# deep-privacy/sidekit

Hardware: AMD Instinct MI355X
Metric: x-vectors/sec (4 s @ 16 kHz) (higher is better)
Workload: dtype bf16; 1 GPU; HalfResNet34 Xtractor.submit / collect (2 whole batches in flight; each batch is the forward of Xtractor.forward(is_eval=True)), bf16 trunk, batch=256 per GPU, synthetic 4 s @ 16 kHz (BASELINE.json configs[1]); batch_per_gpu=256, samples_per_utt=64000, frames_per_utt=401, resident_input_batches=5, parallelism=utterance-sharded x1, lanes=1

## Files before the change

### sidekit_amd/csrc/conv3x3.hip

```cpp
#include "kernels.h"

namespace sk {

template <typename T> __device__ inline void mma_step(f32x16& acc, const uint4& w, const uint4& x);

template <> __device__ inline void mma_step<bf16_t>(f32x16& acc, const uint4& w, const uint4& x) {
  acc = __builtin_amdgcn_mfma_f32_32x32x16_bf16(__builtin_bit_cast(bf16x8, w), __builtin_bit_cast(bf16x8, x), acc, 0, 0, 0);
}
template <> __device__ inline void mma_step<float>(f32x16& acc, const uint4& w, const uint4& x) {
  acc = __builtin_amdgcn_mfma_f32_32x32x2f32(__builtin_bit_cast(float, w.x), __builtin_bit_cast(float, x.x), acc, 0, 0, 0);
  acc = __builtin_amdgcn_mfma_f32_32x32x2f32(__builtin_bit_cast(float, w.y), __builtin_bit_cast(float, x.y), acc, 0, 0, 0);
  acc = __builtin_amdgcn_mfma_f32_32x32x2f32(__builtin_bit_cast(float, w.z), __builtin_bit_cast(float, x.z), acc, 0, 0, 0);
  acc = __builtin_amdgcn_mfma_f32_32x32x2f32(__builtin_bit_cast(float, w.w), __builtin_bit_cast(float, x.w), acc, 0, 0, 0);
}

enum { LANES_LINEAR = 0, LANES_GRID = 1, LANES_DENSE = 2 };
template <typename T_, int CIN_, int COUT_, int S_, int WIN_, int TH_, int WM_, int WN_, int MW_, int NW_, int CK_, int TAPS_, int OCC_ = 0, int PD_ = 0, bool SWZ_ = false, int BLK_ = LANES_LINEAR, bool M16_ = false, bool DIRECT_ = false, bool S2G_ = false, int LEANF_ = -1>
struct ConvCfg {
  static constexpr bool DIRECT = DIRECT_;
  static_assert(!DIRECT_ || (!M16_), "DIRECT: 32x32 MFMA accumulator layout");
  using T = T_;
  static constexpr int EB = elem<T_>::bytes;
  static constexpr int CIN = CIN_, COUT = COUT_, S = S_, WIN = WIN_, TH = TH_, WM = WM_, WN = WN_, MW = MW_, NW = NW_, CK = CK_;
  static constexpr int TAPS = TAPS_;
  static constexpr int WOUT = WIN / S;
  static constexpr int MT = TH * WOUT;
  static constexpr int NT = WN * NW * 32;
  static constexpr int RIN = (TH - 1) * S + 3;
  static constexpr int WP = WIN + 2;
  static constexpr int CB = CK * EB;
  static constexpr bool SWZ = SWZ_;
  static constexpr int BLK = BLK_;
  static constexpr int GC = BLK == LANES_GRID ? (WIN_ / S_) / MW_ : 16, GR = 16 / GC;
  static_assert(BLK == LANES_LINEAR || (SWZ_ && S_ == 1 && TAPS_ == 9), "block lane orders: swizzled image, stride 1, 3x3");
  static_assert(BLK != LANES_GRID || (GC * MW_ == WIN_ / S_ && GR * GC == 16 && TH_ == 2 * WM_ * GR), "GRID: W = MW * GC, TH = 2 * WM * GR");
  static_assert(BLK != LANES_DENSE || (WM_ == 1 && CK_ * elem<T_>::bytes == 256 && TH_ * (WIN_ + 1) <= MW_ * 32), "DENSE: 256-B positions, one wave row");
  static constexpr bool M16 = M16_;
  static_assert(!M16 || ((BLK != LANES_LINEAR || S2G_) && elem<T_>::bytes == 2 && (CK_ * 2) % 64 == 0), "M16: bf16, block lane orders (or the planar stride-2 image), 64-B k-steps");
  static constexpr bool LEAD = BLK == LANES_DENSE || (BLK == LANES_GRID && CK_ * elem<T_>::bytes < 256);
  static constexpr int IMG0 = LEAD ? CK_ * elem<T_>::bytes : 0;
  static constexpr int PSTRIDE = SWZ ? CB : CB + 16;
  static constexpr int SPP = PSTRIDE / 16;
  static constexpr int PPR = ((SWZ ? WIN : WP) * SPP + 63) / 64;
  static constexpr int RS = SWZ ? (WIN + 1) * CB : PPR * 1024;
  static constexpr int LDS_SWZ = (RIN - 1) * RS + (PPR * 1024 > RS ? PPR * 1024 : RS);
  static constexpr int LDS_BLK = BLK == LANES_DENSE ? IMG0 + (MW * 32 + 2 * (WIN + 1) + 2) * CB : IMG0 + LDS_SWZ;
  static constexpr int LDS_IN = BLK ? (LDS_BLK + 255) / 256 * 256 : (SWZ ? (LDS_SWZ + 255) / 256 * 256 : RIN * RS);
  static constexpr int LDS_OUT = TH_ * (WIN_ / S_) * (WN_ * 32 * elem<T_>::bytes + 16);
  static constexpr int LDS = LDS_IN > LDS_OUT ? LDS_IN : (LDS_OUT + 255) / 256 * 256;
  static constexpr int SWF = SPP < 16 ? SPP : 16;
  static constexpr int SWSH = SPP == 4 ? 2 : (SPP == 8 ? 1 : 0);
  static constexpr int KCMASK = (GC >> SWSH) - 1;
  static constexpr int KRSH = SWSH == 0 ? (GC == 4 ? 2 : (GC == 8 ? 3 : 4)) : (SWSH == 1 ? (GC == 8 ? 2 : 3) : 2);
  static constexpr bool S2G = S2G_;
  static constexpr int S2GR = S2G_ ? TH_ / WM_ : 1, S2GC = 16 / S2GR, S2NBC = (WIN_ / S_) / S2GC;
  static constexpr int S2PPB = 256 / (CK_ * elem<T_>::bytes) > 0 ? 256 / (CK_ * elem<T_>::bytes) : 1;
  static constexpr int S2PB = S2GC / S2PPB > 0 ? S2GC / S2PPB : 1;
  static_assert(!S2G_ || (BLK_ == LANES_LINEAR && SWZ_ && S_ == 2 && TAPS_ == 9 && TH_ % WM_ == 0 && S2GR * S2GC == 16 &&
                          (WIN_ / 2) % S2GC == 0 && 2 * MW_ >= S2NBC && S2GC >= S2PPB && S2GR * S2PB == CK_ * elem<T_>::bytes / 16),
                "S2G: stride 2, swizzled image, 16-position blocks that tile the output rows, one key value per slot of a position");
  __host__ __device__ static constexpr int planar(int col) { return (col < 0 || col >= WIN) ? WIN : (col & 1) * (WIN / 2) + (col >> 1); }
  __host__ __device__ static constexpr int unplanar(int P) { return P < WIN / 2 ? 2 * P : 2 * (P - WIN / 2) + 1; }
  __host__ __device__ static constexpr int s2_rowkey(int row) {
    const int hp = (row >> 1) & (S2GR - 1);
    return ((M16_ && S2GR == 8) ? (((hp << 1) & 7) | (hp >> 2)) : hp) * S2PB;
  }
  __host__ __device__ static constexpr int s2p_half(int p) { return (p >= 4 && p < 12) ? 1 : 0; }
  __host__ __device__ static constexpr int s2p_j(int p) { return p < 4 ? p : (p < 12 ? p - 4 : p - 8); }
  __host__ __device__ static constexpr int s2p_row(int p) { return S2GR == 8 ? 2 * (s2p_j(p) / S2GC) + s2p_half(p) : s2p_half(p) * (S2GR / 2) + s2p_j(p) / S2GC; }
  __host__ __device__ static constexpr int s2p_col(int p) { return s2p_j(p) % S2GC; }
  static constexpr int PT16 = S2G_ ? S2NBC : 2 * MW_;
  __host__ __device__ static constexpr int swz_key(int row, int col) {
    if (S2G) return s2_rowkey(row) | ((col / S2PPB) & (S2PB - 1));
    if (BLK == LANES_GRID) return (((row & (GR - 1)) << KRSH) | ((col >> SWSH) & KCMASK)) & (SWF - 1);
    if (BLK == LANES_DENSE) return dense_key((row * (WIN + 1) + col) & 15);
    return (col >> SWSH) & (SWF - 1);
  }
  __host__ __device__ static constexpr int dense_key(int x) { return (M16_ && BLK_ == LANES_DENSE) ? (((x & 7) << 1) | (x >> 3)) : x; }
  __host__ __device__ static constexpr int p16_row(int p) { return GR == 2 ? ((p >= 4 && p < 12) ? 1 : 0) : p / GC; }
  __host__ __device__ static constexpr int p16_col(int p) { return GR == 2 ? (p < 4 ? p : (p < 12 ? p - 4 : p - 8)) : p % GC; }
  __host__ __device__ static constexpr int p16_dense(int p) { return p < 8 ? p : (p < 12 ? p + 4 : p - 4); }
  static_assert(!SWZ || (SPP == 4 || SPP == 8 || SPP == 16 || SPP == 32), "swizzled image: 64..512 B per position");
  static constexpr int KS = CB / 32;
  static constexpr int NCH = CIN / CK;
  static constexpr int KTOT = NCH * TAPS * KS;
  static constexpr int OCC = OCC_ ? OCC_ : ((MW * NW <= 5 && 160 * 1024 / LDS * WM * WN >= 8) ? 2 : 1);
  static constexpr int NK = TAPS * KS;
  static constexpr int KS32 = CB / 64, NK32 = TAPS * KS32, KTOT32 = NCH * NK32;
  static constexpr int MT16 = 2 * MW, NT16 = 2 * NW;
  static constexpr int PD = PD_ ? PD_ : ((NK * NW <= 24) ? NK : (NW == 1 ? 8 : 4));
  static constexpr int PD16 = NK32 * NT16 <= 18 ? NK32 : (PD_ >= 16 ? PD_ - 16 : 2);
  static constexpr bool RESIDENT = TAPS == 9 && NCH == 1 && (M16 ? PD16 == NK32 : PD == NK) && NT == COUT;
  static constexpr bool LEAN = LEANF_ < 0 ? (RESIDENT || OCC >= 3) : (LEANF_ != 0);
  static_assert(MT <= WM * MW * 32, "positions must be covered by the waves' 32-row MFMA tiles (trailing tiles may be partial or idle)");
  static constexpr bool PARTIAL_M = MT < WM * MW * 32;
  __device__ static inline int lane_pos16(int wm, int t, int p) {
    if constexpr (S2G) {
      return t < S2NBC ? (wm * S2GR + s2p_row(p)) * WOUT + t * S2GC + s2p_col(p) : MT;
    } else if constexpr (BLK == LANES_GRID) {
      return ((2 * wm + t / MW) * GR + p16_row(p)) * WOUT + (t % MW) * GC + p16_col(p);
    } else {
      const int L = t * 16 + p16_dense(p), row = L / (WIN + 1), col = L % (WIN + 1);
      return (col < WIN && row < TH) ? row * WOUT + col : MT;
    }
  }
  __device__ static inline int lane_pos(int wm, int i, int r) {
    if constexpr (BLK == LANES_GRID) {
      const int g = ((r >= 4 && r < 12) || (r >= 16 && r < 20) || r >= 28) ? 1 : 0;
      const int j = r - (r < 4 ? 0 : (r < 12 ? 4 : (r < 20 ? 8 : (r < 28 ? 12 : 16))));
      return ((2 * wm + g) * GR + j / GC) * WOUT + i * GC + j % GC;
    } else if constexpr (BLK == LANES_DENSE) {
      const int L = i * 32 + r, row = L / (WIN + 1), col = L % (WIN + 1);
      return (col < WIN && row < TH) ? row * WOUT + col : MT;
    } else if constexpr (S2G) {
      const int g = ((r >= 4 && r < 12) || (r >= 16 && r < 20) || r >= 28) ? 1 : 0;
      const int j = r - (r < 4 ? 0 : (r < 12 ? 4 : (r < 20 ? 8 : (r < 28 ? 12 : 16))));
      const int bc = 2 * i + g;
      return bc < S2NBC ? (wm * S2GR + j / S2GC) * WOUT + bc * S2GC + j % S2GC : MT;
    } else {
      return (wm * MW + i) * 32 + r;
    }
  }
  static_assert(COUT % NT == 0 && CIN % CK == 0 && CB % 32 == 0, "channel tiling");
  static_assert(LDS <= 160 * 1024, "LDS budget");
};

enum { FORM_PLAIN = 0, FORM_STATS = 1, FORM_RESID = 2, FORM_RESID_SC = 3 };
template <int F> struct FormTag { static constexpr int value = F; };

template <class C, int FORM>
__global__ __launch_bounds__(C::WM * C::WN * 64, C::OCC)
void conv3x3_kernel(ConvArgs a) {
  using T = typename C::T;
  constexpr int NWAVES = C::WM * C::WN, NTHREADS = NWAVES * 64;
  constexpr int NY = C::COUT / C::NT;
  const int bidx = NY == 1 ? (int)blockIdx.x : (int)(((blockIdx.x >> 3) / NY) * 8 + (blockIdx.x & 7));
  const int nt0 = (NY == 1 ? 0 : (int)((blockIdx.x >> 3) % NY)) * (C::NT / 32);
  __shared__ __attribute__((aligned(1024))) unsigned char smem[C::LDS];
  const int tid = threadIdx.x, lane = tid & 63, wave = __builtin_amdgcn_readfirstlane(tid >> 6);
  const int r = lane & 31, h = lane >> 5;
  const int wm = __builtin_amdgcn_readfirstlane(wave / C::WN), wn = __builtin_amdgcn_readfirstlane(wave % C::WN);
  const int tiles = (a.Hout + C::TH - 1) / C::TH;
  const int nwork = a.B * tiles, q8 = nwork >> 3, r8 = nwork & 7, xcd = bidx & 7;
  const int wfirst = xcd < r8 ? xcd * (q8 + 1) : r8 * (q8 + 1) + (xcd - r8) * q8, wcount = q8 + (xcd < r8 ? 1 : 0);
  const int wstride = (int)(gridDim.x >> 3) + (xcd < (int)(gridDim.x & 7) ? 1 : 0);
  auto stamp = [&](int k) {
    if (a.stamps && tid == 0) {
      unsigned long long* sp = a.stamps + (size_t)bidx * 8;
      sp[k] = __builtin_amdgcn_s_memtime();
      if (k == 0) sp[7] = __builtin_amdgcn_s_memrealtime();
      if (k == 6) sp[7] = __builtin_amdgcn_s_memrealtime() - sp[7];
    }
  };

  int base[C::BLK ? 1 : C::MW][C::SWZ ? 3 : 1];
  constexpr int NTR = (C::BLK == LANES_GRID && C::GR >= 4) ? 3 : 1;
  int tapreg[C::BLK == LANES_GRID ? NTR : 1][3];
  int fixreg = 0;
  if constexpr (C::BLK == LANES_GRID && C::M16) {
    const int p = lane & 15, q = lane >> 4;
    const int row0 = C::p16_row(p), col0 = C::p16_col(p);
    const int lanebase = (2 * wm * C::GR + row0) * C::RS + col0 * C::CB;
#pragma unroll
    for (int t = 0; t < NTR; ++t)
#pragma unroll
      for (int dw = 0; dw < 3; ++dw) tapreg[t][dw] = lanebase + ((C::swz_key(row0 + t, col0 + dw - 1) ^ q) << 4);
    if constexpr (!C::LEAD) fixreg = col0 == 0 ? C::RS - C::CB : -C::CB;
  } else if constexpr (C::BLK == LANES_GRID) {
    const int g = ((r >= 4 && r < 12) || (r >= 16 && r < 20) || r >= 28) ? 1 : 0;
    const int j = r - (r < 4 ? 0 : (r < 12 ? 4 : (r < 20 ? 8 : (r < 28 ? 12 : 16))));
    const int row0 = (2 * wm + g) * C::GR + j / C::GC, col0 = j % C::GC;
    const int lanebase = row0 * C::RS + col0 * C::CB;
#pragma unroll
    for (int t = 0; t < NTR; ++t)
#pragma unroll
      for (int dw = 0; dw < 3; ++dw) tapreg[t][dw] = lanebase + ((C::swz_key(row0 + t, col0 + dw - 1) ^ h) << 4);
    if constexpr (!C::LEAD) fixreg = col0 == 0 ? C::RS - C::CB : -C::CB;
  }
  int s2x = 0;
  int s2b[3] = {0, 0, 0}, s2bz = 0;
  if constexpr (C::S2G && C::M16) {
    const int p = lane & 15, q = lane >> 4;
    const int ho = wm * C::S2GR + C::s2p_row(p), pcol = C::s2p_col(p);
    s2x = (C::s2_rowkey(2 * ho) ^ C::s2_rowkey(2 * ho + 2)) << 4;
#pragma unroll
    for (int dw = 0; dw < 3; ++dw) {
      const int P = dw == 1 ? pcol : C::WIN / 2 + pcol - (dw == 0 ? 1 : 0);
      s2b[dw] = (2 * ho) * C::RS + P * C::CB + ((q ^ C::swz_key(2 * ho, P)) << 4);
    }
    const int Pz = pcol == 0 ? C::WIN : C::WIN / 2 + pcol - 1;
    s2bz = (2 * ho) * C::RS + Pz * C::CB + ((q ^ C::swz_key(2 * ho, Pz)) << 4);
  }
  if constexpr (C::S2G && !C::M16) {
    const int g = ((r >= 4 && r < 12) || (r >= 16 && r < 20) || r >= 28) ? 1 : 0;
    const int j = r - (r < 4 ? 0 : (r < 12 ? 4 : (r < 20 ? 8 : (r < 28 ? 12 : 16))));
    const int ho = wm * C::S2GR + j / C::S2GC;
    s2x = (C::s2_rowkey(2 * ho) ^ C::s2_rowkey(2 * ho + 2)) << 4;
#pragma unroll
    for (int i = 0; i < C::MW; ++i) {
      const int bc = 2 * i + g < C::S2NBC ? 2 * i + g : C::S2NBC - 1;
      const int wo = bc * C::S2GC + j % C::S2GC;
#pragma unroll
      for (int dw = 0; dw < 3; ++dw) {
        const int P = C::planar(2 * wo + dw - 1);
        base[i][dw] = (2 * ho) * C::RS + P * C::CB + ((h ^ C::swz_key(2 * ho, P)) << 4);
      }
    }
  }
#pragma unroll
  for (int i = 0; i < ((C::BLK || C::S2G) ? 0 : C::MW); ++i) {
    const int mraw = (wm * C::MW + i) * 32 + r, m = (C::PARTIAL_M && mraw >= C::MT) ? C::MT - 1 : mraw;
    const int ho = m / C::WOUT, wo = m % C::WOUT;
    if constexpr (C::SWZ) {
#pragma unroll
      for (int dw = 0; dw < 3; ++dw) {
        int col = wo * C::S + dw - 1;
        if (col < 0) col = C::WIN;
        const int f = (col >> C::SWSH) & (C::SWF - 1);
        base[i][dw] = (ho * C::S) * C::RS + col * C::CB + ((h ^ f) << 4);
      }
    } else {
      base[i][0] = (ho * C::S) * C::RS + (wo * C::S) * C::PSTRIDE + h * 16;
    }
  }
  const unsigned char* wbase = reinterpret_cast<const unsigned char*>(a.wpack);
  const unsigned lane16 = (unsigned)lane * 16u;
  auto wload = [&](int j, int kidx) {
    const unsigned soff = (unsigned)__builtin_amdgcn_readfirstlane(((nt0 + j * C::WN + wn) * C::KTOT + kidx) * 1024);
    return *reinterpret_cast<const uint4*>(wbase + soff + lane16);
  };
  const unsigned char* in = reinterpret_cast<const unsigned char*>(a.in);

  constexpr int NK = C::NK, PD = C::PD;
  constexpr bool RESIDENT = C::RESIDENT;
  auto kord = [](int kk) {
    return (C::SWZ && C::TAPS == 9 && !C::BLK) ? ((kk % 3) * 3 + kk / (3 * C::KS)) * C::KS + (kk / 3) % C::KS : kk;
  };
  uint4 wq[C::M16 ? 1 : PD][C::NW];
  constexpr int PD16 = C::PD16, NK32 = C::NK32;
  uint4 wq16[C::M16 ? PD16 : 1][C::M16 ? C::NT16 : 1];
  auto wload16 = [&](int jn, int kidx32) {
    const unsigned soff = (unsigned)__builtin_amdgcn_readfirstlane(((2 * (nt0 + (jn >> 1) * C::WN + wn) + (jn & 1)) * C::KTOT32 + kidx32) * 1024);
    return *reinterpret_cast<const uint4*>(wbase + soff + lane16);
  };
  auto load_weights = [&](int ch) {
// ... 28 lines not shown
#pragma unroll
  for (int i = 0; i < C::MW; ++i)
#pragma unroll
    for (int j = 0; j < C::NW; ++j)
#pragma unroll
      for (int q = 0; q < 16; ++q) acc[i][j][q] = 0.f;

  for (int ch = 0; ch < C::NCH; ++ch) {
    if constexpr (!RESIDENT) load_weights(ch);
    __builtin_amdgcn_sched_barrier(0);
    if (ch) __syncthreads();
    constexpr int CPP = C::CB / 16, NPIECE = C::RIN * C::PPR;
    if constexpr (C::SWZ) {
      if (ch == 0) {
        for (int s = tid; s < C::RIN * C::SPP; s += NTHREADS)
          *reinterpret_cast<uint4*>(smem + C::IMG0 + (s / C::SPP) * C::RS + C::WIN * C::CB + (s % C::SPP) * 16) = make_uint4(0, 0, 0, 0);
        if constexpr (C::LEAD) {
          if (tid < C::SPP) *reinterpret_cast<uint4*>(smem + tid * 16) = make_uint4(0, 0, 0, 0);
        }
      }
    }
    for (int it = (a.dbg & 4) ? NPIECE : wave; it < NPIECE; it += NWAVES) {
      const int row = it / C::PPR, q = it % C::PPR;
      const int hi = hi0 + row;
      const bool rowok = hi >= 0 && hi < hin_b;
      const unsigned char* rowbase = in + ((((size_t)b * a.Hin + hi) * C::WIN) * C::CIN + ch * C::CK) * C::EB;
      const int slot = q * 64 + lane;
      const unsigned char* src = reinterpret_cast<const unsigned char*>(a.zeros);
      if constexpr (C::SWZ) {
        const int col = slot / C::SPP, cs = slot % C::SPP;
        const int cc = cs ^ C::swz_key(row, col);
        if (rowok) src = rowbase + (C::S2G ? C::unplanar(col) : col) * (C::CIN * C::EB) + cc * 16;
        if ((C::WIN * C::SPP) % 64 == 0 || slot < C::WIN * C::SPP)
          __builtin_amdgcn_global_load_lds((const __attribute__((address_space(1))) void*)src,
                                           (__attribute__((address_space(3))) void*)(smem + C::IMG0 + row * C::RS + q * 1024), 16, 0, 0);
      } else {
        const int col = slot / C::SPP, cc = slot - col * C::SPP;
        if (rowok && cc < CPP && col >= 1 && col <= C::WIN) src = rowbase + (col - 1) * (C::CIN * C::EB) + cc * 16;
        __builtin_amdgcn_global_load_lds((const __attribute__((address_space(1))) void*)src,
                                         (__attribute__((address_space(3))) void*)(smem + it * 1024), 16, 0, 0);
      }
    }
    stamp(1);
    __syncthreads();
    stamp(2);
    __builtin_amdgcn_s_setprio(0);
    auto step_tap = [](int kk) { return (C::SWZ && C::TAPS == 9 && !C::BLK) ? (kk % 3) * 3 + kk / (3 * C::KS) : kk / C::KS; };
    auto step_ks = [](int kk) { return (C::SWZ && C::TAPS == 9 && !C::BLK) ? (kk / 3) % C::KS : kk % C::KS; };
    int rl = r;
    if constexpr (C::BLK == LANES_DENSE) asm volatile("" : "+v"(rl));
    auto xaddr = [&](int i, int kk) {
      const int t = step_tap(kk), ks = step_ks(kk);
      const int tap = (C::TAPS == 9) ? t : 4;
      if constexpr (C::BLK != LANES_LINEAR) {
        const int dh = tap / 3, dw = tap % 3;
        if constexpr (C::BLK == LANES_DENSE) {
          const int v = (rl * C::CB + ((((rl + dh * (C::WIN + 1) + dw - 1) & 15) ^ h) << 4)) ^ (ks << 5);
          return smem + v + (32 * i + dh * (C::WIN + 1) + dw) * C::CB;
        } else {
          const int v = tapreg[NTR == 3 ? dh : 0][dw] ^ ((ks << 5) ^ ((C::GR == 2 && (dh & 1)) ? (16 << C::KRSH) : 0));
          if (!C::LEAD && dw == 0 && i == 0) return smem + (v + fixreg) + dh * C::RS;
          return smem + v + (C::IMG0 + (i * C::GC + dw - 1) * C::CB + dh * C::RS);
        }
      } else if constexpr (C::S2G) return smem + (base[i][tap % 3] ^ ((ks << 5) ^ (tap / 3 == 2 ? s2x : 0))) + (tap / 3) * C::RS;
      else if constexpr (C::SWZ) return smem + (base[i][tap % 3] ^ (ks << 5)) + (tap / 3) * C::RS;
      else return smem + base[i][0] + (tap / 3) * C::RS + (tap % 3) * C::PSTRIDE + ks * 32;
    };
    if constexpr (C::M16) {
      typedef float f32x4v __attribute__((ext_vector_type(4)));
      const int q16 = lane >> 4;
      int pl = C::BLK == LANES_DENSE ? C::p16_dense(lane & 15) : (lane & 15);
      if constexpr (C::BLK == LANES_DENSE) asm volatile("" : "+v"(pl));
      auto xaddr16 = [&](int t, int kk) {
        const int tap = kk / C::KS32, sk = kk % C::KS32, dh = tap / 3, dw = tap % 3;
        if constexpr (C::S2G) {
          const int tt = t < C::PT16 ? t : C::PT16 - 1;
          const int v = ((dw == 0 && tt == 0) ? s2bz : s2b[dw]) ^ ((sk << 6) ^ (dh == 2 ? s2x : 0));
          return smem + v + (tt * C::S2GC * C::CB + dh * C::RS);
        } else if constexpr (C::BLK == LANES_DENSE) {
          const int v = (pl * C::CB + ((C::dense_key((pl + dh * (C::WIN + 1) + dw - 1) & 15) ^ q16) << 4)) ^ (sk << 6);
          return smem + v + (16 * t + dh * (C::WIN + 1) + dw) * C::CB;
        } else {
          const int v = tapreg[NTR == 3 ? dh : 0][dw] ^ ((sk << 6) ^ ((C::GR == 2 && (dh & 1)) ? (16 << C::KRSH) : 0));
          const int brow = (t / C::MW) * C::GR, bcol = (t % C::MW) * C::GC;
          if (!C::LEAD && dw == 0 && bcol == 0) return smem + (v + fixreg) + (brow + dh) * C::RS;
          return smem + v + (C::IMG0 + (bcol + dw - 1) * C::CB + (brow + dh) * C::RS);
        }
      };
      constexpr int HT = C::MW;
      uint4 x16[HT];
#pragma unroll
      for (int t = 0; t < HT; ++t) x16[t] = *reinterpret_cast<const uint4*>(xaddr16(t, 0));
      if (!(a.dbg & 2))
#pragma unroll
      for (int u = 0; u < 2 * NK32; ++u) {
        const int kk = u >> 1, t0 = (u & 1) * HT;
        uint4 wf[C::NT16];
#pragma unroll
        for (int jn = 0; jn < C::NT16; ++jn) wf[jn] = wq16[kk % PD16][jn];
        if ((u & 1) && kk + PD16 < NK32) {
#pragma unroll
          for (int jn = 0; jn < C::NT16; ++jn) wq16[kk % PD16][jn] = wload16(jn, ch * NK32 + kk + PD16);
        }
        __builtin_amdgcn_sched_barrier(0);
#pragma unroll
        for (int t = 0; t < HT; ++t)
#pragma unroll
          for (int jn = 0; jn < C::NT16; ++jn) {
            if (t0 + t >= C::PT16) continue;
            f32x16& A = acc[(t0 + t) >> 1][jn >> 1];
            const int q0 = 4 * (2 * ((t0 + t) & 1) + (jn & 1));
            f32x4v part = {A[q0], A[q0 + 1], A[q0 + 2], A[q0 + 3]};
            part = __builtin_amdgcn_mfma_f32_16x16x32_bf16(__builtin_bit_cast(bf16x8, wf[jn]), __builtin_bit_cast(bf16x8, x16[t]), part, 0, 0, 0);
#pragma unroll
            for (int e = 0; e < 4; ++e) A[q0 + e] = part[e];
          }
        if (u + 1 < 2 * NK32) {
#pragma unroll
          for (int t = 0; t < HT; ++t) x16[t] = *reinterpret_cast<const uint4*>(xaddr16(((u + 1) & 1) * HT + t, (u + 1) >> 1));
        }
      }
      continue;
    }
    uint4 xc[C::MW], xn[C::MW];
#pragma unroll
    for (int i = 0; i < C::MW; ++i) xc[i] = *reinterpret_cast<const uint4*>(xaddr(i, 0));
    if (!(a.dbg & 2))
#pragma unroll
    for (int kk = 0; kk < NK; ++kk) {
      if (kk + 1 < NK && C::OCC < 3) {
#pragma unroll
        for (int i = 0; i < C::MW; ++i) xn[i] = *reinterpret_cast<const uint4*>(xaddr(i, kk + 1));
      }
      uint4 wf[C::NW];
#pragma unroll
      for (int j = 0; j < C::NW; ++j) wf[j] = wq[kk % PD][j];
      if (kk + PD < NK) {
#pragma unroll
        for (int j = 0; j < C::NW; ++j) wq[kk % PD][j] = wload(j, ch * NK + kord(kk + PD));
      }
      __builtin_amdgcn_sched_barrier(0);
#pragma unroll
      for (int i = 0; i < C::MW; ++i)
#pragma unroll
        for (int j = 0; j < C::NW; ++j) mma_step<T>(acc[i][j], wf[j], xc[i]);
      if (kk + 1 < NK) {
#pragma unroll
        for (int i = 0; i < C::MW; ++i) {
          if constexpr (C::OCC < 3) xc[i] = xn[i];
          else xc[i] = *reinterpret_cast<const uint4*>(xaddr(i, kk + 1));
        }
      }
    }
  }

  constexpr int NC = C::WN * 32;
  constexpr int OPS = NC * C::EB + 16;
  static_assert(C::MT * OPS <= C::LDS, "out tile must fit the consumed input buffer");
  if (!(a.dbg & 128)) __builtin_amdgcn_s_setprio(3);
  const int mvalid = (hout_b - ho0) * C::WOUT < C::MT ? (hout_b - ho0) * C::WOUT : C::MT;
  const size_t gpos0 = ((size_t)b * a.Hout + ho0) * C::WOUT;
  auto lds_elem = [&](int m, int c) {
    if constexpr (C::EB == 2) return bf16_to_f32(*reinterpret_cast<const uint16_t*>(smem + m * OPS + c * 2));
    else return *reinterpret_cast<const float*>(smem + m * OPS + c * 4);
  };
  stamp(3);
  auto emit = [&](auto form, auto& accv, const float* scale, const float* shift, unsigned char* out, bool relu) {
// ... 101 lines not shown
    const unsigned char* scut = reinterpret_cast<const unsigned char*>(a.shortcut);
    constexpr int NPRE = (RESID && C::LEAN) ? (NIT + 1) / 2 : NIT;
    uint4 sreg[RESID ? NIT : 1];
    constexpr bool ROWRUN = NC == C::COUT;
    const size_t run0 = gpos0 * C::COUT * C::EB;
    auto fetch_shortcut = [&](int q) {
      const int idx = tid + q * NTHREADS, m = idx / CPR, cc = idx % CPR;
      if constexpr (ROWRUN) return (idx < mvalid * CPR) ? *reinterpret_cast<const uint4*>(scut + run0 + (unsigned)idx * 16u) : make_uint4(0, 0, 0, 0);
      return (idx < mvalid * CPR) ? *reinterpret_cast<const uint4*>(scut + ((gpos0 + m) * C::COUT + nt0 * 32 + j * NC) * C::EB + cc * 16)
                                  : make_uint4(0, 0, 0, 0);
    };
    if constexpr (RESID) {
#pragma unroll
      for (int q = 0; q < NPRE; ++q) sreg[q] = fetch_shortcut(q);
    }
    __syncthreads();
    const int p16 = lane & 15, q16 = lane >> 4;
    auto pos_of = [&](int i, int g) { return C::M16 ? C::lane_pos16(wm, 2 * i + (g >> 1), p16) : C::lane_pos(wm, i, r); };
    auto coff = [&](int g) { return C::M16 ? 16 * (g & 1) + 4 * q16 : 8 * g + 4 * h; };
    constexpr int NSUM = C::M16 ? 8 : 16;
    auto sidx = [](int g) { return C::M16 ? 4 * (g & 1) : 4 * g; };
    float* sp = nullptr;
    if constexpr (STATS) sp = se_part + (((size_t)b * tiles + tile) * C::WM + wm) * C::COUT + nbase;
    float ssum[STATS ? NSUM : 1];
    if constexpr (STATS) {
#pragma unroll
      for (int q = 0; q < NSUM; ++q) ssum[q] = 0.f;
    }
    auto ld4 = [&](const float* p, int g) { return *reinterpret_cast<const f32x4*>(p + nbase + coff(g)); };
    const float* gate_b = (RESID || RSC) ? gate + (size_t)b * C::COUT : scale;
    auto cell = [&](int i, int g, const f32x4& sc, const f32x4& sh, const f32x4& gt, auto full_tag) {
      const int m = pos_of(i, g);
      const bool valid = decltype(full_tag)::value || m < mvalid;
      unsigned char* lp = smem + m * OPS + (wn * 32 + coff(g)) * C::EB;
      const bool store = !C::PARTIAL_M || m < C::MT;
      float v[4];
#pragma unroll
      for (int q = 0; q < 4; ++q) {
        float x = fmaf(accv[i][j][4 * g + q], sc[q], sh[q]);
        if constexpr (STATS) x = relu_nan(x);
        else if constexpr (!RESID) { if (relu) x = relu_nan(x); }
        v[q] = x;
      }
      if constexpr (C::EB == 2) {
        const uint32_t u01 = pack_bf16x2(v[0], v[1]), u23 = pack_bf16x2(v[2], v[3]);
        if constexpr (STATS) {
          const float r[4] = {__builtin_bit_cast(float, u01 << 16), __builtin_bit_cast(float, u01 & 0xffff0000u),
                              __builtin_bit_cast(float, u23 << 16), __builtin_bit_cast(float, u23 & 0xffff0000u)};
#pragma unroll
          for (int q = 0; q < 4; ++q) ssum[sidx(g) + q] += valid ? r[q] : 0.f;
        }
        if (store) *reinterpret_cast<uint2*>(lp) = make_uint2(u01, u23);
      } else {
        if constexpr (STATS) {
#pragma unroll
          for (int q = 0; q < 4; ++q) ssum[sidx(g) + q] += valid ? v[q] : 0.f;
        }
        if (store) *reinterpret_cast<float4*>(lp) = make_float4(v[0], v[1], v[2], v[3]);
      }
    };
    if constexpr (RSC) {
      constexpr int SS = C::COUT == 32 ? 1 : 2, CX = C::COUT == 32 ? 32 : C::COUT / 2;
      constexpr int KX = CX * C::EB / 32;
      const unsigned char* xin = reinterpret_cast<const unsigned char*>(a.sc_in);
      const unsigned char* scb = reinterpret_cast<const unsigned char*>(a.sc_wpack);
      constexpr int KX16 = C::M16 ? CX * C::EB / 64 : 1;
      uint4 wx[C::M16 ? 1 : KX];
      uint4 wx16[C::M16 ? 2 : 1][KX16];
      if constexpr (C::M16) {
#pragma unroll
        for (int n = 0; n < 2; ++n)
#pragma unroll
          for (int sk = 0; sk < KX16; ++sk) {
            const unsigned soff = (unsigned)__builtin_amdgcn_readfirstlane(((2 * (nt0 + j * C::WN + wn) + n) * KX16 + sk) * 1024);
            wx16[n][sk] = *reinterpret_cast<const uint4*>(scb + soff + (unsigned)lane * 16u);
          }
      } else {
#pragma unroll
        for (int ks = 0; ks < KX; ++ks) {
          const unsigned soff = (unsigned)__builtin_amdgcn_readfirstlane(((nt0 + j * C::WN + wn) * KX + ks) * 1024);
          wx[ks] = *reinterpret_cast<const uint4*>(scb + soff + (unsigned)lane * 16u);
        }
      }
#pragma unroll
      for (int g = 0; g < 4; ++g) {
        const f32x4 sc = ld4(scale, g), gt = ld4(gate_b, g);
#pragma unroll
        for (int i = 0; i < C::MW; ++i)
#pragma unroll
          for (int q = 0; q < 4; ++q) accv[i][j][4 * g + q] *= sc[q] * gt[q];
      }
      if constexpr (C::M16) {
        typedef float f32x4v __attribute__((ext_vector_type(4)));
        auto xload16 = [&](int t, uint4* dst) {
          const int m = C::lane_pos16(wm, t, p16);
          const int ho = m / C::WOUT, wo = m % C::WOUT;
          const unsigned char* xp = xin + ((((size_t)b * a.sc_hin + (size_t)(ho0 + ho) * SS) * (C::WOUT * SS) + wo * SS) * CX) * C::EB + q16 * 16;
#pragma unroll
          for (int sk = 0; sk < KX16; ++sk) dst[sk] = (m < mvalid) ? *reinterpret_cast<const uint4*>(xp + sk * 64) : make_uint4(0, 0, 0, 0);
        };
        uint4 xf[KX16], xn[KX16];
        xload16(0, xf);
#pragma unroll
        for (int t = 0; t < C::MT16; ++t) {
          if (t + 1 < C::MT16) xload16(t + 1, xn);
#pragma unroll
          for (int sk = 0; sk < KX16; ++sk)
#pragma unroll
            for (int n = 0; n < 2; ++n) {
              f32x16& A = accv[t >> 1][j];
              const int q0 = 4 * (2 * (t & 1) + n);
              f32x4v part = {A[q0], A[q0 + 1], A[q0 + 2], A[q0 + 3]};
              part = __builtin_amdgcn_mfma_f32_16x16x32_bf16(__builtin_bit_cast(bf16x8, wx16[n][sk]), __builtin_bit_cast(bf16x8, xf[sk]), part, 0, 0, 0);
#pragma unroll
              for (int e = 0; e < 4; ++e) A[q0 + e] = part[e];
            }
#pragma unroll
          for (int sk = 0; sk < KX16; ++sk) xf[sk] = xn[sk];
        }
      }
      constexpr bool AHEAD = KX <= 4;
      auto xload = [&](int i, uint4* dst) {
        const int m = C::lane_pos(wm, i, r);
        const int ho = m / C::WOUT, wo = m % C::WOUT;
        const unsigned char* xp = xin + ((((size_t)b * a.sc_hin + (size_t)(ho0 + ho) * SS) * (C::WOUT * SS) + wo * SS) * CX) * C::EB + h * 16;
#pragma unroll
        for (int ks = 0; ks < KX; ++ks) dst[ks] = (m < mvalid) ? *reinterpret_cast<const uint4*>(xp + ks * 32) : make_uint4(0, 0, 0, 0);
      };
      if constexpr (!C::M16) {
      uint4 xf[KX], xn[AHEAD ? KX : 1];
      xload(0, xf);
#pragma unroll
      for (int i = 0; i < C::MW; ++i) {
        if constexpr (AHEAD) { if (i + 1 < C::MW) xload(i + 1, xn); }
#pragma unroll
        for (int ks = 0; ks < KX; ++ks) mma_step<T>(accv[i][j], wx[ks], xf[ks]);
        if (i + 1 < C::MW) {
          if constexpr (AHEAD) {
#pragma unroll
            for (int ks = 0; ks < KX; ++ks) xf[ks] = xn[ks];
          } else {
            xload(i + 1, xf);
          }
        }
      }
      }
#pragma unroll
      for (int g = 0; g < 4; ++g) {
        const f32x4 sh = ld4(shift, g), gt = ld4(gate_b, g), h2 = ld4(a.sc_shift, g);
#pragma unroll
        for (int i = 0; i < C::MW; ++i) {
          const int m = pos_of(i, g);
          unsigned char* lp = smem + m * OPS + (wn * 32 + coff(g)) * C::EB;
          float v[4];
#pragma unroll
          for (int q = 0; q < 4; ++q) v[q] = relu_nan(accv[i][j][4 * g + q] + (sh[q] * gt[q] + h2[q]));
          if (!C::PARTIAL_M || m < C::MT) {
            if constexpr (C::EB == 2) *reinterpret_cast<uint2*>(lp) = make_uint2(pack_bf16x2(v[0], v[1]), pack_bf16x2(v[2], v[3]));
            else *reinterpret_cast<float4*>(lp) = make_float4(v[0], v[1], v[2], v[3]);
          }
        }
      }
    } else if constexpr (C::LEAN) {
      f32x4 sc_n = ld4(scale, 0), sh_n = ld4(shift, 0), gt_n = ld4(gate_b, 0);
#pragma unroll
      for (int g = 0; g < 4; ++g) {
        const f32x4 sc = sc_n, sh = sh_n, gt = gt_n;
        if (g + 1 < 4) {
          sc_n = ld4(scale, g + 1);
          sh_n = ld4(shift, g + 1);
          if constexpr (RESID) gt_n = ld4(gate_b, g + 1);
        }
        f32x4 sck = sc, shk = sh;
        if constexpr (RESID) {
#pragma unroll
          for (int q = 0; q < 4; ++q) { sck[q] = sc[q] * gt[q]; shk[q] = sh[q] * gt[q]; }
        }
        if (STATS && !C::PARTIAL_M && mvalid == C::MT) {
#pragma unroll
          for (int i = 0; i < C::MW; ++i) cell(i, g, sck, shk, gt, FormTag<1>{});
        } else {
#pragma unroll
          for (int i = 0; i < C::MW; ++i) cell(i, g, sck, shk, gt, FormTag<0>{});
        }
      }
    } else {
      f32x4 sc[4], sh[4], gt[4];
#pragma unroll
      for (int g = 0; g < 4; ++g) {
        sc[g] = ld4(scale, g);
        sh[g] = ld4(shift, g);
        gt[g] = RESID ? ld4(gate_b, g) : sc[g];
        if constexpr (RESID) {
#pragma unroll
          for (int q = 0; q < 4; ++q) { sc[g][q] *= gt[g][q]; sh[g][q] *= gt[g][q]; }
        }
      }
#pragma unroll
      for (int i = 0; i < C::MW; ++i)
#pragma unroll
        for (int g = 0; g < 4; ++g) cell(i, g, sc[g], sh[g], gt[g], FormTag<0>{});
// ... 71 lines not shown
                                  relu_nan(__builtin_bit_cast(float, vv[e] & 0xffff0000u) + __builtin_bit_cast(float, ss[e] & 0xffff0000u)));
            v = make_uint4(rr[0], rr[1], rr[2], rr[3]);
          } else {
            const float4 vf = __builtin_bit_cast(float4, v), sf = __builtin_bit_cast(float4, s);
            v = __builtin_bit_cast(uint4, make_float4(relu_nan(vf.x + sf.x), relu_nan(vf.y + sf.y), relu_nan(vf.z + sf.z), relu_nan(vf.w + sf.w)));
          }
        }
        if constexpr (ROWRUN) *reinterpret_cast<uint4*>(out + run0 + (unsigned)idx * 16u) = v;
        else *reinterpret_cast<uint4*>(out + ((gpos0 + m) * C::COUT + nt0 * 32 + j * NC) * C::EB + cc * 16) = v;
      }
    }
  }
  };
  emit(FormTag<FORM>{}, acc, a.scale, a.shift, reinterpret_cast<unsigned char*>(a.out), a.relu != 0);
  stamp(6);
  return true;
  };
  if constexpr (RESIDENT) {
    bool first_item = true;
    for (int wi = bidx >> 3; wi < wcount; wi += wstride)
      if (do_item(wfirst + wi, first_item)) first_item = false;
  } else {
    if ((bidx >> 3) < wcount) do_item(wfirst + (bidx >> 3), true);
  }
}

static int cu_count() {
  static int n = 0;
  if (!n) {
    int dev = 0, v = 0;
    if (hipGetDevice(&dev) == hipSuccess && hipDeviceGetAttribute(&v, hipDeviceAttributeMultiprocessorCount, dev) == hipSuccess && v > 0) n = v;
    else n = 256;
  }
  return n;
}

template <class C>
static int launch_cfg(const ConvArgs& a, hipStream_t st) {
  const int tiles = cdiv(a.Hout, C::TH), nwork = a.B * tiles;
  constexpr int NWV = C::WM * C::WN;
  const int occ = C::OCC * 4 / NWV, by_lds = 160 * 1024 / C::LDS;
  const int per_cu = (occ < by_lds ? (occ > 0 ? occ : 1) : by_lds);
  const int resident_wgs = cu_count() * ((a.persist_cap > 0 && a.persist_cap < per_cu) ? a.persist_cap : per_cu);
  constexpr int NY = C::COUT / C::NT;
  static_assert(NY == 1 || !C::RESIDENT, "persistent shapes cover all output channels");
  dim3 grid((unsigned)(NY > 1 ? cdiv(nwork, 8) * 8 * NY : ((C::RESIDENT && !(a.dbg & 8) && nwork > resident_wgs) ? resident_wgs : nwork)), 1);
  const dim3 block(NWV * 64);
  if (a.dbg & 16) {
    int nb = -1;
    if constexpr (C::TAPS == 9) (void)hipOccupancyMaxActiveBlocksPerMultiprocessor(&nb, conv3x3_kernel<C, FORM_STATS>, NWV * 64, 0);
    fprintf(stderr, "[conv occupancy] LDS %d B, compiled for %d waves/SIMD: %d workgroups per CU\n", C::LDS, C::OCC, nb);
  }
  SK_CHECK(!(a.gate && a.se_part), SK_EARG, "a convolution is either the statistics or the residual form");
  SK_CHECK(!a.se_part || a.relu, SK_EARG, "the statistics form is conv1 + bn1 + ReLU of a block: relu must be set");
  SK_CHECK(!a.sc_wpack || a.sc_in, SK_EARG, "the 1x1 shortcut weights belong to the in-place shortcut form (sc_in)");
  if constexpr (C::TAPS == 9) {
    if (a.se_part) {
      hipLaunchKernelGGL((conv3x3_kernel<C, FORM_STATS>), grid, block, 0, st, a);
      SK_HIP(hipGetLastError());
      return SK_OK;
    }
    if constexpr (C::S == 1 && C::CIN == C::COUT) {
      if (a.gate && a.sc_in) {
        SK_CHECK(a.sc_wpack && a.sc_scale && a.sc_shift && !a.shortcut, SK_EARG, "in-place shortcut form: bad arguments");
        hipLaunchKernelGGL((conv3x3_kernel<C, FORM_RESID_SC>), grid, block, 0, st, a);
        SK_HIP(hipGetLastError());
        return SK_OK;
      }
    }
    if constexpr (C::S == 1) {
      if (a.gate) {
        hipLaunchKernelGGL((conv3x3_kernel<C, FORM_RESID>), grid, block, 0, st, a);
        SK_HIP(hipGetLastError());
        return SK_OK;
      }
    }
  }
  SK_CHECK(!a.gate && !a.se_part, SK_EARG, "this convolution shape has no statistics / residual form");
  hipLaunchKernelGGL((conv3x3_kernel<C, FORM_PLAIN>), grid, block, 0, st, a);
  SK_HIP(hipGetLastError());
  return SK_OK;
}

using B_L1   = ConvCfg<bf16_t,  32,  32, 1, 80,  8, 4, 1, 5, 1, 32, 9, 0, 0, true>;
using B_L1S  = ConvCfg<bf16_t,  32,  32, 1, 80,  8, 4, 1, 5, 1, 32, 1, 0, 0, true>;
using B_L2A  = ConvCfg<bf16_t,  32,  64, 2, 80,  4, 2, 2, 3, 1, 32, 9, 3, 0, true, LANES_LINEAR, true, false, true>;
using B_L2S  = ConvCfg<bf16_t,  32,  64, 2, 80,  8, 2, 2, 5, 1, 32, 1, 0, 0, true>;
using B_L2   = ConvCfg<bf16_t,  64,  64, 1, 40,  8, 2, 2, 5, 1, 64, 9, 3, 4, true, LANES_GRID, true>;
using B_L3A  = ConvCfg<bf16_t,  64, 128, 2, 40,  4, 1, 4, 3, 1, 64, 9, 2, 0, true, LANES_LINEAR, true, false, true>;
using B_L3S  = ConvCfg<bf16_t,  64, 128, 2, 40,  8, 1, 4, 5, 1, 64, 1>;
using B_L3   = ConvCfg<bf16_t, 128, 128, 1, 20,  8, 1, 4, 5, 1, 128, 9, 3, 4, true, LANES_GRID, true>;
using B_L4A  = ConvCfg<bf16_t, 128, 256, 2, 20,  8, 1, 4, 3, 1, 64, 9, 2, 0, true, LANES_LINEAR, true, false, true>;
using B_L4S  = ConvCfg<bf16_t, 128, 256, 2, 20, 16, 1, 4, 5, 1, 64, 1>;
using B_L4   = ConvCfg<bf16_t, 256, 256, 1, 10, 17, 1, 4, 6, 1, 128, 9, 2, 0, true, LANES_DENSE, true>;

using B_L3T  = ConvCfg<bf16_t, 128, 128, 1, 20,  3, 1, 4, 2, 1, 128, 9, 1, 16 + 12, true, LANES_DENSE, true>;
using B_L4T  = ConvCfg<bf16_t, 256, 256, 1, 10,  2, 1, 4, 1, 1, 128, 9, 1, 16 + 12, true, LANES_DENSE, true>;

using F_L1   = ConvCfg<float,  32,  32, 1, 80,  8, 4, 1, 5, 1, 32, 9, 0, 0, true>;
using F_L1S  = ConvCfg<float,  32,  32, 1, 80,  8, 4, 1, 5, 1, 32, 1, 0, 0, true>;
using F_L2A  = ConvCfg<float,  32,  64, 2, 80,  8, 2, 2, 5, 1, 16, 9, 0, 0, true>;
using F_L2S  = ConvCfg<float,  32,  64, 2, 80,  8, 2, 2, 5, 1, 16, 1, 0, 0, true>;
using F_L2   = ConvCfg<float,  64,  64, 1, 40,  8, 2, 2, 5, 1, 64, 9, 0, 0, true>;
using F_L3A  = ConvCfg<float,  64, 128, 2, 40,  8, 1, 4, 5, 1, 32, 9>;
using F_L3S  = ConvCfg<float,  64, 128, 2, 40,  8, 1, 4, 5, 1, 32, 1>;
using F_L3   = ConvCfg<float, 128, 128, 1, 20,  8, 1, 4, 5, 1, 128, 9>;
using F_L4A  = ConvCfg<float, 128, 256, 2, 20, 16, 1, 4, 5, 2, 32, 9>;
using F_L4S  = ConvCfg<float, 128, 256, 2, 20, 16, 1, 4, 5, 2, 32, 1>;
using F_L4   = ConvCfg<float, 256, 256, 1, 10, 16, 1, 4, 5, 2, 128, 9>;
using F_L3T = F_L3; using F_L4T = F_L4;

template <class C>
static void fill_geom(ConvGeom& g) {
  g.cin = C::CIN; g.cout = C::COUT; g.stride = C::S; g.win = C::WIN; g.th = C::TH; g.wm = C::WM;
  g.ck = C::CK; g.taps = C::TAPS; g.ks = C::KS; g.eb = C::EB; g.nw = C::NW; g.m16 = C::M16 ? 1 : 0;
}

#define SK_CONV_CASES(X) \
  X(CONV_L1, L1) X(CONV_L1S, L1S) X(CONV_L2A, L2A) X(CONV_L2S, L2S) X(CONV_L2, L2) X(CONV_L3A, L3A) \
  X(CONV_L3S, L3S) X(CONV_L3, L3) X(CONV_L4A, L4A) X(CONV_L4S, L4S) X(CONV_L4, L4) X(CONV_L3T, L3T) X(CONV_L4T, L4T)

int conv_geom(int shape, int dtype, ConvGeom* g) {
  switch (shape) {
#define X(id, name)                                              \
  case id:                                                       \
    if (dtype == DT_BF16) fill_geom<B_##name>(*g); else fill_geom<F_##name>(*g); \
    return SK_OK;
    SK_CONV_CASES(X)
#undef X
  }
  set_error("conv_geom: unknown conv shape %d", shape);
  return SK_EARG;
}

int launch_conv(int shape, int dtype, const ConvArgs& a, hipStream_t st) {
  switch (shape) {
#define X(id, name) \
  case id: return dtype == DT_BF16 ? launch_cfg<B_##name>(a, st) : launch_cfg<F_##name>(a, st);
    SK_CONV_CASES(X)
#undef X
  }
  set_error("launch_conv: unknown conv shape %d", shape);
  return SK_EARG;
}

size_t conv_pack_bytes(const ConvGeom& g) { return (size_t)g.cout * g.cin * g.taps * g.eb; }

void conv_pack_weights(const ConvGeom& g, const float* w, int kh_kw, void* dst) {
  if (g.m16) {
    const int nch = g.cin / g.ck, ks32 = g.ck * g.eb / 64, ktot32 = nch * g.taps * ks32;
    for (int n16 = 0; n16 < g.cout / 16; ++n16)
      for (int ch = 0; ch < nch; ++ch)
        for (int t = 0; t < g.taps; ++t) {
          const int tap = (g.taps == 9) ? t : (kh_kw == 9 ? 4 : 0);
          for (int sk = 0; sk < ks32; ++sk) {
            const size_t kidx = (size_t)(ch * g.taps + t) * ks32 + sk;
            for (int lane = 0; lane < 64; ++lane)
              for (int j = 0; j < 8; ++j) {
                const int co = n16 * 16 + (lane & 15), ci = ch * g.ck + sk * 32 + (lane >> 4) * 8 + j;
                reinterpret_cast<uint16_t*>(dst)[(((size_t)n16 * ktot32 + kidx) * 64 + lane) * 8 + j] = f32_to_bf16(w[((size_t)co * g.cin + ci) * kh_kw + tap]);
              }
          }
        }
    return;
  }
  const int KE = 32 / g.eb, nch = g.cin / g.ck, ktot = nch * g.taps * g.ks;
  for (int nt = 0; nt < g.cout / 32; ++nt)
// ... 21 lines not shown
```

Baseline: 44960 x-vectors/s.

## Switch layer-1 conv to 16x16 MFMA grid lane order with configurable block width

Generalizes the GRID lane order so the block width GC can differ from W/MW, giving one block row per wave row with 16x16x32 MFMA. Layer 1 (32->32 channels, 80 wide) now uses this GRID/M16 layout with 8-wide blocks instead of the linear 32x32 path. It also adds a deeper residual-input prefetch that loads half the tiles up front when the kernel is resident. The aim is better LDS bank behaviour and MFMA shape for the small-channel first stage, at the cost of more register pressure from the extra prefetch buffers.

```diff
diff --git a/sidekit_amd/csrc/conv3x3.hip b/sidekit_amd/csrc/conv3x3.hip
--- a/sidekit_amd/csrc/conv3x3.hip
+++ b/sidekit_amd/csrc/conv3x3.hip
@@ -15,7 +15,7 @@
 }
 
 enum { LANES_LINEAR = 0, LANES_GRID = 1, LANES_DENSE = 2 };
-template <typename T_, int CIN_, int COUT_, int S_, int WIN_, int TH_, int WM_, int WN_, int MW_, int NW_, int CK_, int TAPS_, int OCC_ = 0, int PD_ = 0, bool SWZ_ = false, int BLK_ = LANES_LINEAR, bool M16_ = false, bool DIRECT_ = false, bool S2G_ = false, int LEANF_ = -1>
+template <typename T_, int CIN_, int COUT_, int S_, int WIN_, int TH_, int WM_, int WN_, int MW_, int NW_, int CK_, int TAPS_, int OCC_ = 0, int PD_ = 0, bool SWZ_ = false, int BLK_ = LANES_LINEAR, bool M16_ = false, bool DIRECT_ = false, bool S2G_ = false, int LEANF_ = -1, int GC_ = 0>
 struct ConvCfg {
   static constexpr bool DIRECT = DIRECT_;
   static_assert(!DIRECT_ || (!M16_), "DIRECT: 32x32 MFMA accumulator layout");
@@ -31,9 +31,11 @@
   static constexpr int CB = CK * EB;
   static constexpr bool SWZ = SWZ_;
   static constexpr int BLK = BLK_;
-  static constexpr int GC = BLK == LANES_GRID ? (WIN_ / S_) / MW_ : 16, GR = 16 / GC;
+  static constexpr int GC = BLK == LANES_GRID ? (GC_ ? GC_ : (WIN_ / S_) / MW_) : 16, GR = 16 / GC;
+  static constexpr int NBC = BLK == LANES_GRID ? (WIN_ / S_) / GC : MW_, BRW = 2 * MW_ / NBC;
   static_assert(BLK == LANES_LINEAR || (SWZ_ && S_ == 1 && TAPS_ == 9), "block lane orders: swizzled image, stride 1, 3x3");
-  static_assert(BLK != LANES_GRID || (GC * MW_ == WIN_ / S_ && GR * GC == 16 && TH_ == 2 * WM_ * GR), "GRID: W = MW * GC, TH = 2 * WM * GR");
+  static_assert(BLK != LANES_GRID || (GC * NBC == WIN_ / S_ && GR * GC == 16 && TH_ == BRW * WM_ * GR && BRW * NBC == 2 * MW_ && (BRW == 2 || M16_)),
+                "GRID: W = NBC * GC, TH = BRW * WM * GR, 2 * MW blocks per wave row (one block row per wave row: 16x16x32 only)");
   static_assert(BLK != LANES_DENSE || (WM_ == 1 && CK_ * elem<T_>::bytes == 256 && TH_ * (WIN_ + 1) <= MW_ * 32), "DENSE: 256-B positions, one wave row");
   static constexpr bool M16 = M16_;
   static_assert(!M16 || ((BLK != LANES_LINEAR || S2G_) && elem<T_>::bytes == 2 && (CK_ * 2) % 64 == 0), "M16: bf16, block lane orders (or the planar stride-2 image), 64-B k-steps");
@@ -51,7 +53,7 @@
   static constexpr int SWF = SPP < 16 ? SPP : 16;
   static constexpr int SWSH = SPP == 4 ? 2 : (SPP == 8 ? 1 : 0);
   static constexpr int KCMASK = (GC >> SWSH) - 1;
-  static constexpr int KRSH = SWSH == 0 ? (GC == 4 ? 2 : (GC == 8 ? 3 : 4)) : (SWSH == 1 ? (GC == 8 ? 2 : 3) : 2);
+  static constexpr int KRSH = SWSH == 0 ? (GC == 4 ? 2 : (GC == 8 ? 3 : 4)) : (SWSH == 1 ? (GC == 8 ? 2 : 3) : (GC == 8 ? 1 : 2));
   static constexpr bool S2G = S2G_;
   static constexpr int S2GR = S2G_ ? TH_ / WM_ : 1, S2GC = 16 / S2GR, S2NBC = (WIN_ / S_) / S2GC;
   static constexpr int S2PPB = 256 / (CK_ * elem<T_>::bytes) > 0 ? 256 / (CK_ * elem<T_>::bytes) : 1;
@@ -98,7 +100,7 @@
     if constexpr (S2G) {
       return t < S2NBC ? (wm * S2GR + s2p_row(p)) * WOUT + t * S2GC + s2p_col(p) : MT;
     } else if constexpr (BLK == LANES_GRID) {
-      return ((2 * wm + t / MW) * GR + p16_row(p)) * WOUT + (t % MW) * GC + p16_col(p);
+      return ((BRW * wm + t / NBC) * GR + p16_row(p)) * WOUT + (t % NBC) * GC + p16_col(p);
     } else {
       const int L = t * 16 + p16_dense(p), row = L / (WIN + 1), col = L % (WIN + 1);
       return (col < WIN && row < TH) ? row * WOUT + col : MT;
@@ -160,7 +162,7 @@
   if constexpr (C::BLK == LANES_GRID && C::M16) {
     const int p = lane & 15, q = lane >> 4;
     const int row0 = C::p16_row(p), col0 = C::p16_col(p);
-    const int lanebase = (2 * wm * C::GR + row0) * C::RS + col0 * C::CB;
+    const int lanebase = (C::BRW * wm * C::GR + row0) * C::RS + col0 * C::CB;
 #pragma unroll
     for (int t = 0; t < NTR; ++t)
 #pragma unroll
@@ -355,7 +357,7 @@
           return smem + v + (16 * t + dh * (C::WIN + 1) + dw) * C::CB;
         } else {
           const int v = tapreg[NTR == 3 ? dh : 0][dw] ^ ((sk << 6) ^ ((C::GR == 2 && (dh & 1)) ? (16 << C::KRSH) : 0));
-          const int brow = (t / C::MW) * C::GR, bcol = (t % C::MW) * C::GC;
+          const int brow = (t / C::NBC) * C::GR, bcol = (t % C::NBC) * C::GC;
           if (!C::LEAD && dw == 0 && bcol == 0) return smem + (v + fixreg) + (brow + dh) * C::RS;
           return smem + v + (C::IMG0 + (bcol + dw - 1) * C::CB + (brow + dh) * C::RS);
         }
@@ -623,6 +625,20 @@
           wx[ks] = *reinterpret_cast<const uint4*>(scb + soff + (unsigned)lane * 16u);
         }
       }
+      auto xload16 = [&](int t, uint4* dst) {
+        const int m = C::lane_pos16(wm, t, p16);
+        const int ho = m / C::WOUT, wo = m % C::WOUT;
+        const unsigned char* xp = xin + ((((size_t)b * a.sc_hin + (size_t)(ho0 + ho) * SS) * (C::WOUT * SS) + wo * SS) * CX) * C::EB + q16 * 16;
+#pragma unroll
+        for (int sk = 0; sk < KX16; ++sk) dst[sk] = (m < mvalid) ? *reinterpret_cast<const uint4*>(xp + sk * 64) : make_uint4(0, 0, 0, 0);
+      };
+      constexpr bool XALL = C::M16 && C::RESIDENT && C::MT16 * KX16 <= 10;
+      constexpr int XD = XALL ? C::MT16 / 2 : 1;
+      uint4 xs16[XD][KX16];
+      if constexpr (XALL) {
+#pragma unroll
+        for (int t = 0; t < XD; ++t) xload16(t, xs16[t]);
+      }
 #pragma unroll
       for (int g = 0; g < 4; ++g) {
         const f32x4 sc = ld4(scale, g), gt = ld4(gate_b, g);
@@ -633,18 +649,11 @@
       }
       if constexpr (C::M16) {
         typedef float f32x4v __attribute__((ext_vector_type(4)));
-        auto xload16 = [&](int t, uint4* dst) {
-          const int m = C::lane_pos16(wm, t, p16);
-          const int ho = m / C::WOUT, wo = m % C::WOUT;
-          const unsigned char* xp = xin + ((((size_t)b * a.sc_hin + (size_t)(ho0 + ho) * SS) * (C::WOUT * SS) + wo * SS) * CX) * C::EB + q16 * 16;
-#pragma unroll
-          for (int sk = 0; sk < KX16; ++sk) dst[sk] = (m < mvalid) ? *reinterpret_cast<const uint4*>(xp + sk * 64) : make_uint4(0, 0, 0, 0);
-        };
         uint4 xf[KX16], xn[KX16];
-        xload16(0, xf);
+        if constexpr (!XALL) xload16(0, xf);
 #pragma unroll
         for (int t = 0; t < C::MT16; ++t) {
-          if (t + 1 < C::MT16) xload16(t + 1, xn);
+          if (!XALL && t + 1 < C::MT16) xload16(t + 1, xn);
 #pragma unroll
           for (int sk = 0; sk < KX16; ++sk)
 #pragma unroll
@@ -652,12 +661,16 @@
               f32x16& A = accv[t >> 1][j];
               const int q0 = 4 * (2 * (t & 1) + n);
               f32x4v part = {A[q0], A[q0 + 1], A[q0 + 2], A[q0 + 3]};
-              part = __builtin_amdgcn_mfma_f32_16x16x32_bf16(__builtin_bit_cast(bf16x8, wx16[n][sk]), __builtin_bit_cast(bf16x8, xf[sk]), part, 0, 0, 0);
+              part = __builtin_amdgcn_mfma_f32_16x16x32_bf16(__builtin_bit_cast(bf16x8, wx16[n][sk]), __builtin_bit_cast(bf16x8, XALL ? xs16[t % XD][sk] : xf[sk]), part, 0, 0, 0);
 #pragma unroll
               for (int e = 0; e < 4; ++e) A[q0 + e] = part[e];
             }
-#pragma unroll
-          for (int sk = 0; sk < KX16; ++sk) xf[sk] = xn[sk];
+          if constexpr (XALL) {
+            if (t + XD < C::MT16) xload16(t + XD, xs16[t % XD]);
+          } else {
+#pragma unroll
+            for (int sk = 0; sk < KX16; ++sk) xf[sk] = xn[sk];
+          }
         }
       }
       constexpr bool AHEAD = KX <= 4;
@@ -895,7 +908,7 @@
   return SK_OK;
 }
 
-using B_L1   = ConvCfg<bf16_t,  32,  32, 1, 80,  8, 4, 1, 5, 1, 32, 9, 0, 0, true>;
+using B_L1   = ConvCfg<bf16_t,  32,  32, 1, 80,  8, 4, 1, 5, 1, 32, 9, 0, 0, true, LANES_GRID, true, false, false, -1, 8>;
 using B_L1S  = ConvCfg<bf16_t,  32,  32, 1, 80,  8, 4, 1, 5, 1, 32, 1, 0, 0, true>;
 using B_L2A  = ConvCfg<bf16_t,  32,  64, 2, 80,  4, 2, 2, 3, 1, 32, 9, 3, 0, true, LANES_LINEAR, true, false, true>;
 using B_L2S  = ConvCfg<bf16_t,  32,  64, 2, 80,  8, 2, 2, 5, 1, 32, 1, 0, 0, true>;
```

Result: no change. 45350 x-vectors/s (median of 6 runs) (+0.9%).
